# gaetanfacchinetti/DensityFlows.jl

Hardware: AMD Instinct MI355X
Metric: forward+logdetJ Msamples/s, d=5 8-layer RealNVP, 1/2/4/8 MI355X (higher is better)
Workload: dtype f32

## Files before the change

densityflows.jl_amd/csrc/df_uniform_impl.h:

```cpp
#pragma once

#include <type_traits>

#include "df_chain_impl.h"

namespace df {
namespace uni {


using impl::lds4;
using impl::mfma4;
using impl::Stager;

__device__ __forceinline__ float relu_fast(float x) {
    return __int_as_float(__builtin_elementwise_max(__float_as_int(x), 0));
}

__device__ __forceinline__ float xgroup_sum(float p) {
    auto a = __builtin_amdgcn_permlane16_swap(__float_as_uint(p), __float_as_uint(p), false, false);
    const float q = __uint_as_float(a[0]) + __uint_as_float(a[1]);
    auto b = __builtin_amdgcn_permlane32_swap(__float_as_uint(q), __float_as_uint(q), false, false);
    return __uint_as_float(b[0]) + __uint_as_float(b[1]);
}


template <int HT, int TT, int KS = 0>
__device__ __forceinline__ void dense_first(const uint8_t* buf, const UNet& N, const float (&xin)[TT][4],
                                            f32x4 (&acc)[TT][HT]) {
    const int lane = threadIdx.x & 63;
    const float* wb = reinterpret_cast<const float*>(buf + N.off_w0) + lane;
    const int ks = KS > 0 ? KS : N.ks;
    if constexpr (KS > 0) {
#pragma unroll
        for (int m = 0; m < HT; ++m) {
            const float w = wb[m * KS * 64];
#pragma unroll
            for (int t = 0; t < TT; ++t) acc[t][m] = mfma4(w, xin[t][0], f32x4{0.f, 0.f, 0.f, 0.f});
        }
#pragma unroll
        for (int r = 1; r < KS; ++r)
#pragma unroll
            for (int m = 0; m < HT; ++m) {
                const float w = wb[(m * KS + r) * 64];
#pragma unroll
                for (int t = 0; t < TT; ++t) acc[t][m] = mfma4(w, xin[t][r], acc[t][m]);
            }
        return;
    }
#pragma unroll
    for (int t = 0; t < TT; ++t)
#pragma unroll
        for (int m = 0; m < HT; ++m) acc[t][m] = f32x4{0.f, 0.f, 0.f, 0.f};
#pragma unroll
    for (int r = 0; r < 4; ++r) {
        if (r < ks) {
#pragma unroll
            for (int m = 0; m < HT; ++m) {
                const float w = wb[(m * ks + r) * 64];
#pragma unroll
                for (int t = 0; t < TT; ++t) acc[t][m] = mfma4(w, xin[t][r], acc[t][m]);
            }
        }
    }
}

template <int HT, int TT>
__device__ __forceinline__ void dense_hidden(const uint8_t* wb, const f32x4 (&in)[TT][HT], f32x4 (&out)[TT][HT]) {
    const int lane = threadIdx.x & 63;
    wb += lane * 16;
    constexpr int MB = HT < 2 ? HT : 2;
#pragma unroll
    for (int t = 0; t < TT; ++t)
#pragma unroll
        for (int m = 0; m < HT; ++m) out[t][m] = f32x4{0.f, 0.f, 0.f, 0.f};
#pragma unroll
    for (int m0 = 0; m0 < HT; m0 += MB) {
        f32x4 w[2][MB];
#pragma unroll
        for (int mm = 0; mm < MB; ++mm) w[0][mm] = lds4(wb + (m0 + mm) * 1024);
#pragma unroll
        for (int kq = 0; kq < HT; ++kq) {
            const int cb = kq & 1;
            if (kq + 1 < HT) {
#pragma unroll
                for (int mm = 0; mm < MB; ++mm) w[cb ^ 1][mm] = lds4(wb + ((kq + 1) * HT + m0 + mm) * 1024);
            }
#pragma unroll
            for (int r = 0; r < 4; ++r)
#pragma unroll
                for (int mm = 0; mm < MB; ++mm)
#pragma unroll
                    for (int t = 0; t < TT; ++t)
                        out[t][m0 + mm] = mfma4(w[cb][mm][r], in[t][kq][r], out[t][m0 + mm]);
        }
    }
}

template <int HT, int TT, bool RELU>
__device__ __forceinline__ void bias_act(const uint8_t* bb, int act, f32x4 (&v)[TT][HT], bool add_bias = true) {
    const int g = (threadIdx.x & 63) >> 4;
    if (add_bias) {
#pragma unroll
        for (int m = 0; m < HT; ++m) {
            const f32x4 b = lds4(bb + ((16 * m + 4 * g) << 2));
#pragma unroll
            for (int t = 0; t < TT; ++t) v[t][m] = v[t][m] + b;
        }
    }
    if (RELU || act == DF_ACT_RELU) {
#pragma unroll
        for (int t = 0; t < TT; ++t)
#pragma unroll
            for (int m = 0; m < HT; ++m)
#pragma unroll
                for (int r = 0; r < 4; ++r) v[t][m][r] = relu_fast(v[t][m][r]);
    } else if (act != DF_ACT_IDENTITY) {
        if (!RELU) {
#pragma unroll
            for (int t = 0; t < TT; ++t)
#pragma unroll
                for (int m = 0; m < HT; ++m)
#pragma unroll
                    for (int r = 0; r < 4; ++r) v[t][m][r] = impl::act_fn(act, v[t][m][r]);
        }
    }
}

template <int HT, int TT, bool RELU, int NO = 0>
__device__ __forceinline__ void out_valu(const uint8_t* buf, const UNet& N, const f32x4 (&h)[TT][HT],
                                         f32x4 (&o)[TT]) {
    const int g = (threadIdx.x & 63) >> 4;
    const uint8_t* w3 = buf + N.off_out;
    constexpr int INP = 16 * HT;
    const int n_out = NO > 0 ? NO : N.n_out;
    const float* b3 = reinterpret_cast<const float*>(w3) + n_out * INP;
#pragma unroll
    for (int t = 0; t < TT; ++t) o[t] = f32x4{0.f, 0.f, 0.f, 0.f};
#pragma unroll
    for (int oo = 0; oo < 4; ++oo) {
        if (oo < n_out) {
            float p[TT];
#pragma unroll
            for (int t = 0; t < TT; ++t) p[t] = 0.f;
#pragma unroll
            for (int kq = 0; kq < HT; ++kq) {
                const f32x4 w = lds4(w3 + ((oo * INP + 16 * kq + 4 * g) << 2));
#pragma unroll
                for (int r = 0; r < 4; ++r)
#pragma unroll
                    for (int t = 0; t < TT; ++t) p[t] = __builtin_fmaf(w[r], h[t][kq][r], p[t]);
            }
            const float bo = b3[oo];
#pragma unroll
            for (int t = 0; t < TT; ++t) {
                const float v = xgroup_sum(p[t]) + bo;
                o[t][oo] = (RELU || N.act_out == DF_ACT_IDENTITY) ? v : impl::act_fn(N.act_out, v);
            }
        }
    }
}

template <int HT, int TT, int NO>
__device__ __forceinline__ void out_valu_t(const uint8_t* buf, const UNet& N, const f32x4 (&h)[TT][HT],
                                           float (&y)[TT]) {
    static_assert(NO >= 1 && NO <= 4, "FAST tails: 1..4 outputs");
    const int g = (threadIdx.x & 63) >> 4;
    const uint8_t* w3 = buf + N.off_out;
    constexpr int INP = 16 * HT;
    float p[TT][4];
#pragma unroll
    for (int t = 0; t < TT; ++t)
#pragma unroll
        for (int oo = 0; oo < 4; ++oo) p[t][oo] = 0.f;
#pragma unroll
    for (int oo = 0; oo < NO; ++oo)
#pragma unroll
        for (int kq = 0; kq < HT; ++kq) {
            const f32x4 w = lds4(w3 + ((oo * INP + 16 * kq + 4 * g) << 2));
#pragma unroll
            for (int r = 0; r < 4; ++r)
#pragma unroll
                for (int t = 0; t < TT; ++t) p[t][oo] = __builtin_fmaf(w[r], h[t][kq][r], p[t][oo]);
        }
    const float bo = reinterpret_cast<const float*>(w3)[NO * INP + (g < NO ? g : 0)];
#pragma unroll
    for (int t = 0; t < TT; ++t) {
        auto a = __builtin_amdgcn_permlane16_swap(__float_as_uint(p[t][0]), __float_as_uint(p[t][1]), false, false);
        const float A = __uint_as_float(a[0]) + __uint_as_float(a[1]);
        float Bv = 0.f;
        if constexpr (NO > 2) {
            auto b = __builtin_amdgcn_permlane16_swap(__float_as_uint(p[t][2]), __float_as_uint(p[t][3]), false, false);
            Bv = __uint_as_float(b[0]) + __uint_as_float(b[1]);
        }
        auto c = __builtin_amdgcn_permlane32_swap(__float_as_uint(A), __float_as_uint(Bv), false, false);
        y[t] = (__uint_as_float(c[0]) + __uint_as_float(c[1])) + bo;
    }
}

template <int NO>
__device__ __forceinline__ float group_row_sum(float y) {
    float s = y;
    if constexpr (NO > 1) {
        auto a = __builtin_amdgcn_permlane16_swap(__float_as_uint(y), __float_as_uint(y), false, false);
        s = s + __uint_as_float(a[1]);
    }
    if constexpr (NO > 2) {
        auto b = __builtin_amdgcn_permlane32_swap(__float_as_uint(y), __float_as_uint(y), false, false);
        const float y2 = __uint_as_float(b[1]);
        s = s + y2;
        if constexpr (NO > 3) {
            auto c = __builtin_amdgcn_permlane16_swap(__float_as_uint(y2), __float_as_uint(y2), false, false);
            s = s + __uint_as_float(c[1]);
        }
    }
    return s;
}

template <int HT, int TT, bool RELU>
__device__ __forceinline__ void out_mfma(const uint8_t* buf, const UNet& N, const f32x4 (&h)[TT][HT],
                                         f32x4 (&out)[TT][2]) {
    const int lane = threadIdx.x & 63, g = lane >> 4;
    const uint8_t* wb = buf + N.off_out + lane * 16;
    const int mt = (N.n_out + 15) >> 4;
#pragma unroll
    for (int t = 0; t < TT; ++t) out[t][0] = out[t][1] = f32x4{0.f, 0.f, 0.f, 0.f};
#pragma unroll
    for (int kq = 0; kq < HT; ++kq) {
        const f32x4 w0 = lds4(wb + (kq * mt + 0) * 1024);
#pragma unroll
        for (int r = 0; r < 4; ++r)
#pragma unroll
            for (int t = 0; t < TT; ++t) out[t][0] = mfma4(w0[r], h[t][kq][r], out[t][0]);
        if (mt > 1) {
            const f32x4 w1 = lds4(wb + (kq * mt + 1) * 1024);
#pragma unroll
            for (int r = 0; r < 4; ++r)
#pragma unroll
                for (int t = 0; t < TT; ++t) out[t][1] = mfma4(w1[r], h[t][kq][r], out[t][1]);
        }
    }
    const uint8_t* bb = buf + N.off_out + HT * mt * 1024;
#pragma unroll
    for (int m = 0; m < 2; ++m) {
        if (m < mt) {
            const f32x4 b = lds4(bb + ((16 * m + 4 * g) << 2));
#pragma unroll
            for (int t = 0; t < TT; ++t) {
                f32x4 v = out[t][m] + b;
                if (!RELU && N.act_out != DF_ACT_IDENTITY)
#pragma unroll
                    for (int r = 0; r < 4; ++r) v[r] = impl::act_fn(N.act_out, v[r]);
                out[t][m] = v;
            }
        }
    }
}

template <int PH>
__device__ __forceinline__ float couple1(float v, float y) {
    if (PH == impl::PH_S_FWD) return v * expf(y);
    if (PH == impl::PH_T_FWD) return v + y;
    if (PH == impl::PH_T_BWD) return v - y;
    return v * expf(-y);
}

template <int HT, int TT, bool OUTV, bool RELU, int PH, int NO = 0>
__device__ __forceinline__ void tail(const uint8_t* buf, const UNet& N, const ULayer& L, const int32_t* tab,
                                     float* state, const int (&ro)[TT], float (&sum)[TT], const f32x4 (&H)[TT][HT]) {
    const int g = (threadIdx.x & 63) >> 4;
    constexpr bool SPH = (PH == impl::PH_S_FWD || PH == impl::PH_S_BWD);
    const int32_t* af = tab + L.af_tab;
    const int n_af = (OUTV && NO > 0) ? NO : L.n_af;
#pragma unroll
    for (int t = 0; t < TT; ++t) sum[t] = 0.f;
#ifdef DF_EXP_NOTAIL
    if (true) {
#pragma unroll
        for (int t = 0; t < TT; ++t) {
            float acc = 0.f;
#pragma unroll
            for (int m = 0; m < HT; ++m) acc += H[t][m][0];
            asm volatile("" ::"v"(acc));
        }
        return;
    }
#endif
    if constexpr (OUTV && NO > 0) {
        float y[TT];
        out_valu_t<HT, TT, NO>(buf, N, H, y);
        const int slot = af[g < NO ? g : 0];
#pragma unroll
        for (int t = 0; t < TT; ++t) {
            if (g < NO) state[ro[t] + slot] = couple1<PH>(state[ro[t] + slot], y[t]);
            if (SPH) sum[t] = group_row_sum<NO>(y[t]);
        }
    } else if constexpr (OUTV) {
        f32x4 o[TT];
        out_valu<HT, TT, RELU, NO>(buf, N, H, o);
        const int slot = (g < n_af) ? af[g] : 0;
#pragma unroll
        for (int t = 0; t < TT; ++t) {
            const float y = impl::sel4(o[t], g);
            if (g < n_af) state[ro[t] + slot] = couple1<PH>(state[ro[t] + slot], y);
            if (SPH) {
                float s_ = o[t][0];
#pragma unroll
                for (int oo = 1; oo < 4; ++oo)
                    if (oo < n_af) s_ = s_ + o[t][oo];
                sum[t] = s_;
            }
        }
    } else {
        f32x4 o[TT][2];
        out_mfma<HT, TT, RELU>(buf, N, H, o);
#pragma unroll
        for (int t = 0; t < TT; ++t) {
            float p = 0.f;
#pragma unroll
            for (int m = 0; m < 2; ++m)
#pragma unroll
                for (int r = 0; r < 4; ++r) {
                    const int oo = 16 * m + 4 * g + r;
                    if (oo < L.n_af) {
                        const int slot = af[oo];
                        const float y = o[t][m][r];
                        state[ro[t] + slot] = couple1<PH>(state[ro[t] + slot], y);
                        if (SPH) p = p + y;
                    }
                }
            if (SPH) sum[t] = xgroup_sum(p);
        }
    }
}

typedef __bf16 bf16x8 __attribute__((ext_vector_type(8)));

__device__ __forceinline__ f32x4 mfma_bf(const bf16x8& a, const bf16x8& b, f32x4 c) {
    return __builtin_amdgcn_mfma_f32_16x16x32_bf16(a, b, c, 0, 0, 0);
}

typedef __bf16 bf16x2 __attribute__((ext_vector_type(2)));
#ifndef DF_SPLIT_DOT2
#define DF_SPLIT_DOT2 1
#endif
template <int S>
__device__ __forceinline__ float split_rem(bf16x2 h, float x) {
#if DF_SPLIT_DOT2 == 2
    const uint32_t u = __builtin_bit_cast(uint32_t, h);
    const float hi = __uint_as_float(S == 0 ? (u << 16) : (u & 0xffff0000u));
    float r;
    asm("v_sub_f32 %0, %1, %2" : "=v"(r) : "v"(x), "v"(hi));
    return r;
#elif DF_SPLIT_DOT2
    uint32_t c;
    if (S == 0) asm("v_mov_b32 %0, 0xbf80" : "=v"(c));
    else c = 0xbf800000u;
    return __builtin_amdgcn_fdot2_f32_bf16(h, __builtin_bit_cast(bf16x2, c), x, false);
#else
    return x - (float)h[S];
#endif
}

__device__ __forceinline__ void split2(float a, float b, bf16x2& p0, bf16x2& p1, bf16x2& p2) {
    p0 = bf16x2{(__bf16)a, (__bf16)b};
    const float ra = split_rem<0>(p0, a), rb = split_rem<1>(p0, b);
    p1 = bf16x2{(__bf16)ra, (__bf16)rb};
    p2 = bf16x2{(__bf16)split_rem<0>(p1, ra), (__bf16)split_rem<1>(p1, rb)};
}

__device__ __forceinline__ void split8(const float (&v)[8], bf16x8& p0, bf16x8& p1, bf16x8& p2) {
#pragma unroll
    for (int e = 0; e < 8; e += 2) {
        bf16x2 h, m, l;
        split2(v[e], v[e + 1], h, m, l);
        p0[e] = h[0]; p0[e + 1] = h[1];
        p1[e] = m[0]; p1[e + 1] = m[1];
        p2[e] = l[0]; p2[e + 1] = l[1];
    }
}

#ifndef DF_SPLIT_MREM
#define DF_SPLIT_MREM 1
#endif
typedef short short4v __attribute__((ext_vector_type(4)));
typedef __bf16 bf16x4v __attribute__((ext_vector_type(4)));

__device__ __forceinline__ short4v neg_eye() {
    const int i = threadIdx.x & 3;
    short4v p;
#pragma unroll
    for (int e = 0; e < 4; ++e) p[e] = (e == i) ? (short)0xbf80 : (short)0;
    return p;
}

__device__ __forceinline__ f32x4 mrem(short4v eye, bf16x4v h, f32x4 c) {
    return __builtin_amdgcn_mfma_f32_4x4x4bf16_1k(eye, __builtin_bit_cast(short4v, h), c, 0, 0, 0);
}

__device__ __forceinline__ void split8_mrem(short4v eye, const f32x4& a, const f32x4& b, bf16x8& p0, bf16x8& p1,
                                            bf16x8& p2) {
    bf16x4v h0, h1;
#pragma unroll
    for (int e = 0; e < 4; ++e) {
        h0[e] = (__bf16)a[e];
        h1[e] = (__bf16)b[e];
    }
    p0 = __builtin_shufflevector(h0, h1, 0, 1, 2, 3, 4, 5, 6, 7);
    const f32x4 ra = mrem(eye, h0, a), rb = mrem(eye, h1, b);
#pragma unroll
    for (int e = 0; e < 4; ++e) {
        h0[e] = (__bf16)ra[e];
        h1[e] = (__bf16)rb[e];
    }
    p1 = __builtin_shufflevector(h0, h1, 0, 1, 2, 3, 4, 5, 6, 7);
    const f32x4 sa = mrem(eye, h0, ra), sb = mrem(eye, h1, rb);
#pragma unroll
    for (int e = 0; e < 4; ++e) {
        h0[e] = (__bf16)sa[e];
        h1[e] = (__bf16)sb[e];
    }
    p2 = __builtin_shufflevector(h0, h1, 0, 1, 2, 3, 4, 5, 6, 7);
}

template <int HT, int TT>
__device__ __forceinline__ void dense_first_split(const uint8_t* buf, const UNet& N, const float (&xin)[TT][4],
                                                  f32x4 (&acc)[TT][HT]) {
    const int lane = threadIdx.x & 63;
    bf16x8 b[TT];
    const __bf16 z = (__bf16)0.f;
#pragma unroll
    for (int t = 0; t < TT; t += 2) {
        bf16x2 h, m, l;
        split2(xin[t][0], t + 1 < TT ? xin[t + 1][0] : 0.f, h, m, l);
        b[t] = bf16x8{h[0], m[0], h[0], l[0], m[0], h[0], z, z};
        if (t + 1 < TT) b[t + 1] = bf16x8{h[1], m[1], h[1], l[1], m[1], h[1], z, z};
    }
    const uint8_t* wb = buf + N.off_w0 + lane * 16;
#pragma unroll
    for (int m = 0; m < HT; ++m) {
        const bf16x8 w = *reinterpret_cast<const bf16x8*>(wb + m * 1024);
#pragma unroll
        for (int t = 0; t < TT; ++t) acc[t][m] = mfma_bf(w, b[t], f32x4{0.f, 0.f, 0.f, 0.f});
    }
}

template <int HT, int TT, bool BIAS = true, bool FENCE = false>
__device__ __forceinline__ void dense_hidden_split(const uint8_t* wb, const f32x4 (&in)[TT][HT],
                                                   f32x4 (&out)[TT][HT]) {
    const int lane = threadIdx.x & 63, g = lane >> 4;
    const uint8_t* bb = wb + (HT / 2) * HT * 3072;
    wb += lane * 16;
    const short4v eye = DF_SPLIT_MREM ? neg_eye() : short4v{0, 0, 0, 0};
#pragma unroll
    for (int m = 0; m < HT; ++m) {
        const f32x4 b = BIAS ? lds4(bb + ((16 * m + 4 * g) << 2)) : f32x4{0.f, 0.f, 0.f, 0.f};
#pragma unroll
        for (int t = 0; t < TT; ++t) out[t][m] = b;
    }
#pragma unroll
    for (int c = 0; c < HT / 2; ++c) {
        bf16x8 x[TT][3];
#pragma unroll
        for (int t = 0; t < TT; ++t) {
            const float v[8] = {in[t][2 * c][0],     in[t][2 * c][1],     in[t][2 * c][2],     in[t][2 * c][3],
                                in[t][2 * c + 1][0], in[t][2 * c + 1][1], in[t][2 * c + 1][2], in[t][2 * c + 1][3]};
#ifdef DF_DIAG_NOSPLIT
            for (int e = 0; e < 8; ++e) x[t][0][e] = (__bf16)v[e];
            x[t][1] = x[t][0];
            x[t][2] = x[t][0];
#else
            if constexpr (DF_SPLIT_MREM) split8_mrem(eye, in[t][2 * c], in[t][2 * c + 1], x[t][0], x[t][1], x[t][2]);
            else split8(v, x[t][0], x[t][1], x[t][2]);
#endif
        }
#pragma unroll
        for (int m = 0; m < HT; ++m) {
            const uint8_t* f = wb + (c * HT + m) * 3072;
            const bf16x8 w0 = *reinterpret_cast<const bf16x8*>(f);
            const bf16x8 w1 = *reinterpret_cast<const bf16x8*>(f + 1024);
            const bf16x8 w2 = *reinterpret_cast<const bf16x8*>(f + 2048);
#pragma unroll
            for (int t = 0; t < TT; ++t) {
                f32x4 a = out[t][m];
                a = mfma_bf(w2, x[t][0], a);
                a = mfma_bf(w1, x[t][1], a);
                a = mfma_bf(w0, x[t][2], a);
                a = mfma_bf(w1, x[t][0], a);
                a = mfma_bf(w0, x[t][1], a);
                out[t][m] = mfma_bf(w0, x[t][0], a);
            }
            if (FENCE) asm volatile("" ::: "memory");
        }
    }
}

#ifndef DF_SPLIT_PREFETCH
#define DF_SPLIT_PREFETCH 1
#endif

__device__ __forceinline__ void sched_fence() { __builtin_amdgcn_sched_barrier(0); }

__device__ __forceinline__ void lds_wait0() { __builtin_amdgcn_s_waitcnt(0xc07f); }

struct SplitStep {
    bf16x8 w0, w1, w2;
    f32x4 b;
};

template <int HT, bool BIAS>
__device__ __forceinline__ void split_step_request(const uint8_t* wl, const uint8_t* bl, int s, SplitStep& f) {
    if (s >= (HT / 2) * HT) return;
    const uint8_t* p = wl + s * 3072;
    f.w0 = *reinterpret_cast<const bf16x8*>(p);
    f.w1 = *reinterpret_cast<const bf16x8*>(p + 1024);
    f.w2 = *reinterpret_cast<const bf16x8*>(p + 2048);
    if (BIAS && s < HT) f.b = lds4(bl + (s << 6));
}

template <int HT, int TT, bool BIAS = true>
__device__ __forceinline__ void dense_hidden_split_pf(const uint8_t* wb, int l16, int g16, const f32x4 (&in)[TT][HT],
                                                      f32x4 (&out)[TT][HT], const SplitStep& f0) {
    const uint8_t* bl = wb + (HT / 2) * HT * 3072 + g16;
    const uint8_t* wl = wb + l16;
    const short4v eye = neg_eye();
    SplitStep f[2];
    f[0] = f0;
    bf16x8 x[TT][3];
#pragma unroll
    for (int s = 0; s < (HT / 2) * HT; ++s) {
        const int c = s / HT, m = s % HT;
        if (m == 0) {
#pragma unroll
            for (int t = 0; t < TT; ++t) split8_mrem(eye, in[t][2 * c], in[t][2 * c + 1], x[t][0], x[t][1], x[t][2]);
        }
        constexpr int NS = (HT / 2) * HT;
        const bool late = (m == HT - 1) && (s + 1 < NS);
        sched_fence();
        lds_wait0();
        if (!late) split_step_request<HT, BIAS>(wl, bl, s + 1, f[(s + 1) & 1]);
        sched_fence();
        const SplitStep& w = f[s & 1];
#pragma unroll
        for (int t = 0; t < TT; ++t) {
            f32x4 a = c == 0 ? (BIAS ? w.b : f32x4{0.f, 0.f, 0.f, 0.f}) : out[t][m];
            a = mfma_bf(w.w2, x[t][0], a);
            a = mfma_bf(w.w1, x[t][1], a);
            a = mfma_bf(w.w0, x[t][2], a);
            a = mfma_bf(w.w1, x[t][0], a);
            a = mfma_bf(w.w0, x[t][1], a);
            out[t][m] = mfma_bf(w.w0, x[t][0], a);
        }
        if (late) {
#pragma unroll
            for (int t = 0; t < TT; ++t) asm volatile("" : "+v"(out[t][m]));
            sched_fence();
            split_step_request<HT, BIAS>(wl, bl, s + 1, f[(s + 1) & 1]);
        }
    }
}

template <int HT, int TT>
__device__ __forceinline__ void dense_first_split_pf(const bf16x8 (&w)[HT], const float (&xin)[TT][4],
                                                     f32x4 (&acc)[TT][HT]) {
    bf16x8 b[TT];
    const __bf16 z = (__bf16)0.f;
#pragma unroll
    for (int t = 0; t < TT; ++t) {
        bf16x2 h, m, l;
        h = bf16x2{(__bf16)xin[t][0], z};
        const float r1 = split_rem<0>(h, xin[t][0]);
        m = bf16x2{(__bf16)r1, z};
        l = bf16x2{(__bf16)split_rem<0>(m, r1), z};
        b[t] = bf16x8{h[0], m[0], h[0], l[0], m[0], h[0], z, z};
    }
#pragma unroll
    for (int m = 0; m < HT; ++m)
#pragma unroll
        for (int t = 0; t < TT; ++t) acc[t][m] = mfma_bf(w[m], b[t], f32x4{0.f, 0.f, 0.f, 0.f});
}

template <int HT, int NO>
__device__ __forceinline__ void out_row_request(const uint8_t* w3g, int oo, f32x4 (&w)[HT]) {
    if (oo >= NO) return;
#pragma unroll
    for (int kq = 0; kq < HT; ++kq) w[kq] = lds4(w3g + ((oo * 16 * HT + 16 * kq) << 2));
}

constexpr int split_tail_rows(int TT, int NO) { return (TT == 2 && NO <= 2) ? 1 : TT; }

template <int TT>
struct SplitTail {
    int ce, l16, g16;
    int row[TT];
    float e_old[TT], a_old[TT];
};

template <int HT, int TT, int NO, bool LDJ, int NU>
__device__ __forceinline__ void out_valu_t_pf(const uint8_t* w3g, const f32x4 (&w0)[HT], float bo,
                                              const f32x4 (&h)[TT][HT], const float* state, const int& aslot,
                                              SplitTail<TT>& tl, float (&v)[NU], float (&y)[NU]) {
    static_assert(NO >= 1 && NO <= 4, "FAST tails: 1..4 outputs");
    static_assert(NU == split_tail_rows(TT, NO), "rows a lane group owns");
    float p[TT][4];
#pragma unroll
    for (int t = 0; t < TT; ++t)
#pragma unroll
        for (int oo = 0; oo < 4; ++oo) p[t][oo] = 0.f;
    f32x4 w[2][HT];
#pragma unroll
    for (int kq = 0; kq < HT; ++kq) w[0][kq] = w0[kq];
#pragma unroll
    for (int oo = 0; oo < NO; ++oo) {
        sched_fence();
        lds_wait0();
        if (oo == 0) {
#pragma unroll
            for (int u = 0; u < NU; ++u) {
                v[u] = state[tl.row[u] + aslot];
                if constexpr (LDJ) {
                    tl.e_old[u] = state[tl.row[u] + tl.ce];
                    tl.a_old[u] = state[tl.row[u] + tl.ce - 1];
                }
            }
        }
        out_row_request<HT, NO>(w3g, oo + 1, w[(oo + 1) & 1]);
        sched_fence();
#pragma unroll
        for (int kq = 0; kq < HT; ++kq)
#pragma unroll
            for (int r = 0; r < 4; ++r)
#pragma unroll
                for (int t = 0; t < TT; ++t) p[t][oo] = __builtin_fmaf(w[oo & 1][kq][r], h[t][kq][r], p[t][oo]);
#pragma unroll
        for (int t = 0; t < TT; ++t) asm volatile("" : "+v"(p[t][oo]));
    }
    if constexpr (NU < TT) {
        const float q = NO == 2 ? p[0][1] : p[1][0];
        auto a = __builtin_amdgcn_permlane16_swap(__float_as_uint(p[0][0]), __float_as_uint(q), false, false);
        const float A = __uint_as_float(a[0]) + __uint_as_float(a[1]);
        float Bv = A;
        if constexpr (NO == 2) {
            auto b = __builtin_amdgcn_permlane16_swap(__float_as_uint(p[1][0]), __float_as_uint(p[1][1]), false, false);
            Bv = __uint_as_float(b[0]) + __uint_as_float(b[1]);
        }
        auto c = __builtin_amdgcn_permlane32_swap(__float_as_uint(A), __float_as_uint(Bv), false, false);
        y[0] = (__uint_as_float(c[0]) + __uint_as_float(c[1])) + bo;
    } else {
#pragma unroll
        for (int t = 0; t < TT; ++t) {
            auto a = __builtin_amdgcn_permlane16_swap(__float_as_uint(p[t][0]), __float_as_uint(p[t][1]), false, false);
            const float A = __uint_as_float(a[0]) + __uint_as_float(a[1]);
            float Bv = 0.f;
            if constexpr (NO > 2) {
                auto b = __builtin_amdgcn_permlane16_swap(__float_as_uint(p[t][2]), __float_as_uint(p[t][3]), false, false);
                Bv = __uint_as_float(b[0]) + __uint_as_float(b[1]);
            }
            auto c = __builtin_amdgcn_permlane32_swap(__float_as_uint(A), __float_as_uint(Bv), false, false);
            y[t] = (__uint_as_float(c[0]) + __uint_as_float(c[1])) + bo;
        }
    }
}

struct SplitHead {
    int off_w0, feat_word, af_word;
};
#if DF_SPLIT_PREFETCH && !defined(DF_EXP_NOTAIL) && !defined(DF_DIAG_NOSPLIT)
#define DF_SPLIT_HEAD_REGS 1
#else
#define DF_SPLIT_HEAD_REGS 0
#endif

#ifndef DF_SPLIT_PRIO
#define DF_SPLIT_PRIO 1
#endif
template <bool MATRIX_PHASE>
__device__ __forceinline__ void split_prio() {
    if constexpr (DF_SPLIT_PRIO == 1) __builtin_amdgcn_s_setprio(MATRIX_PHASE ? 2 : 0);
    if constexpr (DF_SPLIT_PRIO == 2) __builtin_amdgcn_s_setprio(MATRIX_PHASE ? 0 : 2);
}

template <int HT, int TT, bool OUTV, bool RELU, int PH, bool FAST = false, int NO = 0, bool SPLIT = false,
          bool LDJ = false, bool LANES = false>
__device__ __forceinline__ void net_tiles(const uint8_t* buf, const UNet& N, const ULayer& L, const int32_t* tab,
                                          float* state, const int (&ro)[TT], float (&sum)[TT], const SplitHead& hd,
                                          SplitTail<TT>& tl) {
    const int lane = threadIdx.x & 63, g = lane >> 4;
    constexpr bool SPH = (PH == impl::PH_S_FWD || PH == impl::PH_S_BWD);
#if DF_SPLIT_HEAD_REGS
    if constexpr (SPLIT && FAST && HT >= 2 && OUTV && NO > 0) {
        int l16 = tl.l16, g16 = tl.g16;
        if constexpr (!LANES) {
            int tx = threadIdx.x;
            asm volatile("" : "+v"(tx));
            l16 = (tx & 63) << 4, g16 = tx & 48;
        }
        const int g = g16 >> 4;
        const uint8_t* net = buf + hd.off_w0;
        const int slot = ((uint32_t)hd.feat_word >> (g16 >> 1)) & ((1 << kSplitSlotBits) - 1);
        static_assert(kSplitSlotBits == 8, "slot of lane group g at bit 8 g = g16 / 2");
        bf16x8 w0[HT];
#pragma unroll
        for (int m = 0; m < HT; ++m) w0[m] = *reinterpret_cast<const bf16x8*>(net + l16 + m * 1024);
        float xin[TT][4];
#pragma unroll
        for (int t = 0; t < TT; ++t) xin[t][0] = state[ro[t] + slot];
        const uint8_t* wh = net + kSplitOffH(HT);
        SplitStep f0;
        split_step_request<HT, true>(wh + l16, wh + (HT / 2) * HT * 3072 + g16, 0, f0);
        sched_fence();
        lds_wait0();
        split_prio<true>();
        sched_fence();
        f32x4 A[TT][HT], B[TT][HT];
        dense_first_split_pf<HT, TT>(w0, xin, A);
        bias_act<HT, TT, true>(buf, DF_ACT_RELU, A, false);
        dense_hidden_split_pf<HT, TT>(wh, l16, g16, A, B, f0);
        const uint8_t* w3 = net + kSplitOffOut(HT);
        const uint8_t* w3g = w3 + g16;
        sched_fence();
        split_prio<false>();
        f32x4 wo[HT];
        out_row_request<HT, NO>(w3g, 0, wo);
        constexpr int NU = split_tail_rows(TT, NO);
        constexpr bool ONE_TREE = NU < TT;
        const int go = ONE_TREE ? (NO == 2 ? (g & 1) : 0) : (g < NO ? g : 0);
        const float bo = reinterpret_cast<const float*>(w3)[NO * 16 * HT + go];
        const int aslot = ((uint32_t)hd.af_word >> (kSplitSlotBits * go)) & ((1 << kSplitSlotBits) - 1);
        if constexpr (ONE_TREE) {
            tl.row[0] = ro[0] + ((NO == 2 ? (g >> 1) : (g & 1)) ? ro[1] - ro[0] : 0);
        } else {
#pragma unroll
            for (int t = 0; t < TT; ++t) tl.row[t] = ro[t];
        }
        sched_fence();
        bias_act<HT, TT, true>(buf, DF_ACT_RELU, B, false);
        float v[NU], y[NU];
        out_valu_t_pf<HT, TT, NO, SPH && LDJ>(w3g, wo, bo, B, state, aslot, tl, v, y);
        if (ONE_TREE || g < NO) {
#pragma unroll
            for (int u = 0; u < NU; ++u) state[tl.row[u] + aslot] = couple1<PH>(v[u], y[u]);
        }
#pragma unroll
        for (int u = 0; u < NU; ++u) {
            if constexpr (!SPH) {
                sum[u] = 0.f;
            } else if constexpr (ONE_TREE && NO == 2) {
                auto a = __builtin_amdgcn_permlane16_swap(__float_as_uint(y[u]), __float_as_uint(y[u]), false, false);
                sum[u] = __uint_as_float(a[0]) + __uint_as_float(a[1]);
            } else if constexpr (ONE_TREE) {
                sum[u] = y[u];
            } else {
                sum[u] = group_row_sum<NO>(y[u]);
            }
        }
        return;
    }
#endif
    if constexpr (SPLIT && FAST && HT >= 2) {
        float xin[TT][4];
        const int slot = tab[L.feat_tab + g];
#pragma unroll
        for (int t = 0; t < TT; ++t) xin[t][0] = state[ro[t] + slot];
        f32x4 A[TT][HT], B[TT][HT];
        dense_first_split<HT, TT>(buf, N, xin, A);
        bias_act<HT, TT, true>(buf, DF_ACT_RELU, A, false);
        dense_hidden_split<HT, TT>(buf + N.off_h, A, B);
        bias_act<HT, TT, true>(buf, DF_ACT_RELU, B, false);
        tail<HT, TT, OUTV, RELU, PH, NO>(buf, N, L, tab, state, ro, sum, B);
        return;
    }
    float xin[TT][4];
    const int32_t* feat = tab + L.feat_tab;
    constexpr int KS = FAST ? 1 : 0;
    const int ks = FAST ? 1 : N.ks;
#pragma unroll
    for (int r = 0; r < 4; ++r) {
        const int slot = (r < ks) ? feat[4 * r + g] : 0;
#pragma unroll
        for (int t = 0; t < TT; ++t) xin[t][r] = (r < ks) ? state[ro[t] + slot] : 0.f;
    }

    f32x4 A[TT][HT], B[TT][HT];
    dense_first<HT, TT, KS>(buf, N, xin, A);
    bias_act<HT, TT, RELU>(buf + N.off_b0, N.act0, A, FAST ? false : !N.fold0);
    if (FAST || N.nh == 1) {
        dense_hidden<HT, TT>(buf + N.off_h, A, B);
        bias_act<HT, TT, RELU>(buf + N.off_h + HT * HT * 1024, N.acth, B);
        tail<HT, TT, OUTV, RELU, PH, NO>(buf, N, L, tab, state, ro, sum, B);
        return;
    }
    bool in_a = true;
    for (int k = 0; k < N.nh; k += 2) {
        dense_hidden<HT, TT>(buf + N.off_h + k * N.hstride, A, B);
        bias_act<HT, TT, RELU>(buf + N.off_h + k * N.hstride + HT * HT * 1024, N.acth, B);
        in_a = false;
        if (k + 1 < N.nh) {
            dense_hidden<HT, TT>(buf + N.off_h + (k + 1) * N.hstride, B, A);
            bias_act<HT, TT, RELU>(buf + N.off_h + (k + 1) * N.hstride + HT * HT * 1024, N.acth, A);
            in_a = true;
        }
    }
    if (in_a) tail<HT, TT, OUTV, RELU, PH, NO>(buf, N, L, tab, state, ro, sum, A);
    else tail<HT, TT, OUTV, RELU, PH, NO>(buf, N, L, tab, state, ro, sum, B);
}

template <int HT, int TT, bool RELU, bool FWDP, int NO>
__device__ __forceinline__ void net_pair_tiles(const uint8_t* buf, const ULayer& L, const int32_t* tab, float* state,
                                               const int (&ro)[TT], float (&ssum)[TT]) {
    const int lane = threadIdx.x & 63, g = lane >> 4;
    float xin[TT][4];
    const int slot_in = tab[L.feat_tab + g];
#pragma unroll
    for (int t = 0; t < TT; ++t) xin[t][0] = state[ro[t] + slot_in];
    f32x4 As[TT][HT], At[TT][HT], Bs[TT][HT], Bt[TT][HT];
    dense_first<HT, TT, 1>(buf, L.s, xin, As);
    dense_first<HT, TT, 1>(buf, L.t, xin, At);
    bias_act<HT, TT, RELU>(buf + L.s.off_b0, L.s.act0, As, false);
    bias_act<HT, TT, RELU>(buf + L.t.off_b0, L.t.act0, At, false);
    dense_hidden<HT, TT>(buf + L.s.off_h, As, Bs);
    dense_hidden<HT, TT>(buf + L.t.off_h, At, Bt);
    bias_act<HT, TT, RELU>(buf + L.s.off_h + HT * HT * 1024, L.s.acth, Bs);
    bias_act<HT, TT, RELU>(buf + L.t.off_h + HT * HT * 1024, L.t.acth, Bt);
    float ys[TT], yt[TT];
    out_valu_t<HT, TT, NO>(buf, L.s, Bs, ys);
    out_valu_t<HT, TT, NO>(buf, L.t, Bt, yt);
    const int slot = tab[L.af_tab + (g < NO ? g : 0)];
#pragma unroll
    for (int t = 0; t < TT; ++t) {
        if (g < NO) {
            float v = state[ro[t] + slot];
            if (FWDP) {
                v = v * expf(ys[t]);
                v = v + yt[t];
            } else {
                v = v - yt[t];
                v = v * expf(-ys[t]);
            }
            state[ro[t] + slot] = v;
        }
        ssum[t] = group_row_sum<NO>(ys[t]);
    }
}

}

#ifndef DF_UNI_WAVES
#define DF_UNI_WAVES 4
#endif
#ifndef DF_FAST_WAVES
#define DF_FAST_WAVES 4
#endif

template <int HT, int MODE, bool OUTV, bool RELU, bool FAST = false, bool SPLIT = false>
__global__ void __launch_bounds__(kBlockThreads, FAST ? DF_FAST_WAVES : DF_UNI_WAVES)
uniform_kernel(ChainArgs a) {
    using namespace uni;
    constexpr bool FWD = (MODE == MODE_FWD || MODE == MODE_FWD_INPLACE);
    constexpr bool WANT_LDJ = (MODE != MODE_FWD_INPLACE);

    extern __shared__ __attribute__((aligned(16))) uint8_t smem[];
    const int stage_area = a.stage_bytes * a.n_stage_bufs;
    int32_t* tab = reinterpret_cast<int32_t*>(smem + stage_area);
    float* state = reinterpret_cast<float*>(smem + stage_area + a.tab_bytes);

    ClockStamp clk;
    clk.begin(a);
#ifdef DF_PHASE_STAMPS
    uint64_t ph[16] = {};
#define DF_PH(i) do { if (blockIdx.x == 0 && threadIdx.x == 0) ph[i] = __builtin_amdgcn_s_memtime(); } while (0)
#else
#define DF_PH(i) do {} while (0)
#endif
    DF_PH(0);
    const int tid = threadIdx.x;
    const int lane = tid & 63, wave = tid >> 6;
    const int g = lane >> 4, j = lane & 15;
    const int d = a.d, n = a.n, stride = a.stride, nd = n + d;
    const int nt = a.tiles;
    const int S = kWavesPerBlock * 16 * nt;
    const int cA = nd + 1, cE = nd + 2;
    const int64_t s0 = (int64_t)blockIdx.x * S;
    const int nvalid = (int)((a.batch - s0) < S ? (a.batch - s0) : S);

    Stager sg;
    sg.base = smem;
    sg.bytes = a.stage_bytes;
    sg.sched = FWD ? a.sched_fwd : a.sched_bwd;
    sg.n = FWD ? a.n_sched_fwd : a.n_sched_bwd;
    constexpr bool kLaneLocalDma = SPLIT && DF_SPLIT_PREFETCH;
    constexpr bool kSplitHead = SPLIT && FAST && OUTV && HT >= 2 && DF_SPLIT_HEAD_REGS;
    impl::stager_start<kLaneLocalDma>(sg, a);

    float* tabf = reinterpret_cast<float*>(tab);
    constexpr int kRowMax = 8;
    const bool fast_copy = d <= kRowMax && n <= kRowMax && a.n_par <= kBlockThreads && a.tab_ints <= 4 * kBlockThreads;
    auto row_init = [&](int smp) {
        for (int c = nd; c < stride; ++c) state[smp * stride + c] = (c == nd + 3) ? 1.f : 0.f;
    };
    auto theta_in = [&](float v, float lo, float hi) {
        const float diff = hi - lo;
        return (diff == 0.f) ? 0.f : (v - lo) / diff;
    };
    if (fast_copy) {
        const int n_tab = a.tab_ints, n_par = a.n_par;
        int tv[4];
#pragma unroll
        for (int u = 0; u < 4; ++u) {
            const int i = tid + u * kBlockThreads;
            tv[u] = i < n_tab ? a.tables[i] : 0;
        }
        const float pv = tid < n_par ? a.params[tid] : 0.f;
        const bool norm_th = a.tmin != nullptr;
        const float blo = (norm_th && lane < n) ? a.tmin[lane] : 0.f;
        const float bhi = (norm_th && lane < n) ? a.tmax[lane] : 0.f;
        const int smp = tid;
        const bool valid = smp < nvalid;
        float zr[kRowMax], tr[kRowMax];
#pragma unroll
        for (int c = 0; c < kRowMax; ++c)
            if (c < d) zr[c] = valid ? a.zin[(s0 + smp) * d + c] : 0.f;
#pragma unroll
        for (int c = 0; c < kRowMax; ++c)
            if (c < n) tr[c] = valid ? a.theta[(s0 + smp) * n + c] : 0.f;
#pragma unroll
        for (int u = 0; u < 4; ++u) {
            const int i = tid + u * kBlockThreads;
            if (i < n_tab) tab[i] = tv[u];
        }
        if (tid < n_par) tabf[n_tab + tid] = pv;
#pragma unroll
        for (int c = 0; c < kRowMax; ++c)
            if (c < n) {
                const float lo = __shfl(blo, c), hi = __shfl(bhi, c);
                if (smp < S) state[smp * stride + c] = (norm_th && valid) ? theta_in(tr[c], lo, hi) : tr[c];
            }
        if (smp < S) {
#pragma unroll
            for (int c = 0; c < kRowMax; ++c)
                if (c < d) state[smp * stride + n + c] = zr[c];
            row_init(smp);
        }
        for (int i = tid + kBlockThreads * d; i < S * d; i += kBlockThreads) {
            const int r = i / d, c = i - r * d;
            state[r * stride + n + c] = r < nvalid ? a.zin[(s0 + r) * d + c] : 0.f;
        }
        for (int i = tid + kBlockThreads * n; i < S * n; i += kBlockThreads) {
            const int r = i / n, c = i - r * n;
            float v = 0.f;
            if (r < nvalid) {
                v = a.theta[(s0 + r) * n + c];
                if (norm_th) v = theta_in(v, a.tmin[c], a.tmax[c]);
            }
            state[r * stride + c] = v;
        }
        for (int r = tid + kBlockThreads; r < S; r += kBlockThreads) row_init(r);
    } else {
        for (int i = tid; i < a.tab_ints; i += kBlockThreads) tab[i] = a.tables[i];
        for (int i = tid; i < S * d; i += kBlockThreads) {
            const int smp = i / d, c = i - smp * d;
            float v = 0.f;
            if (smp < nvalid) v = a.zin[(s0 + smp) * d + c];
            state[smp * stride + n + c] = v;
        }
        for (int i = tid; i < S * n; i += kBlockThreads) {
            const int smp = i / n, c = i - smp * n;
            float v = 0.f;
            if (smp < nvalid) {
                v = a.theta[(s0 + smp) * n + c];
                if (a.tmin) v = theta_in(v, a.tmin[c], a.tmax[c]);
            }
            state[smp * stride + c] = v;
        }
        for (int i = tid; i < S; i += kBlockThreads) row_init(i);
    }
    DF_PH(1);
    DF_PH(2);
    DF_PH(3);
    __syncthreads();
    DF_PH(4);

    const int row0 = ((wave * nt) * 16 + j) * stride;
#ifdef DF_NO_PAIR
    constexpr bool no_pair = true;
#else
    constexpr bool no_pair = false;
#endif
    const int tstep = 16 * stride;
    bool have_acc = false;
    constexpr bool kHoldLanes = kSplitHead && HT == 4 && FWD;
    int lane16 = lane << 4, group16 = g << 4;
    if constexpr (kHoldLanes) asm volatile("" : "+v"(lane16), "+v"(group16));

    auto ldj_update = [&](int ro, float l, bool first_in_elem, bool last_in_elem) {
        if (!WANT_LDJ || g != 0) return;
        const float e = first_in_elem ? l : state[ro + cE] + l;
        state[ro + cE] = e;
        if (last_in_elem) state[ro + cA] = have_acc ? state[ro + cA] + e : e;
    };

    for (int it = 0; it < a.n_layers; ++it) {
        const int li = FWD ? it : a.n_layers - 1 - it;
        using CULayer = const __attribute__((address_space(4))) ULayer;
#ifdef DF_PHASE_STAMPS
        const ULayer L = *(const ULayer*)(&((CULayer*)(uintptr_t)a.ulayers)[li]);
        asm volatile("s_waitcnt lgkmcnt(0)" ::: "memory");
        if (it == 1) DF_PH(13);
#else
        const ULayer& L = *(const ULayer*)(&((CULayer*)(uintptr_t)a.ulayers)[li]);
#endif
        const int kind = L.kind;
        const bool first_in_elem = FWD ? L.elem_start : L.elem_end;
        const bool last_in_elem = FWD ? L.elem_end : L.elem_start;
        int gl = g, jl = j, wavel = wave, row0l = row0;
        if constexpr (kLaneLocalDma) {
            if (kind == DF_LAYER_NORM || (!FWD && a.snap)) {
                int tx = tid;
                asm volatile("" : "+v"(tx));
                gl = (tx & 63) >> 4, jl = tx & 15, wavel = tx >> 6;
                row0l = ((wavel * nt) * 16 + jl) * stride;
            }
        }
        if (kind == DF_LAYER_NORM) {
            const float al = L.alpha, be = L.beta, delta = be - al;
            auto norm = [&](const auto* xmn) {
                const auto* xmx = xmn + d;
                for (int tt = 0; tt < nt; ++tt) {
                    const int ro = row0l + tt * tstep;
                    for (int i = gl; i < d; i += 4) {
                        const float lo = xmn[i], hi = xmx[i], xd = hi - lo;
                        float v = state[ro + n + i];
                        if (FWD) v = ((xd * v - al * hi) + be * lo) / delta;
                        else v = (be * (v - lo) + al * (hi - v)) / xd;
                        state[ro + n + i] = v;
                    }
                    ldj_update(ro, FWD ? L.ldj_const : -L.ldj_const, first_in_elem, last_in_elem);
                }
            };
            if (fast_copy) norm(tabf + a.tab_ints + L.norm_off);
            else norm(a.params + L.norm_off);
        } else {
            const bool rnvp = (kind == DF_LAYER_RNVP);
            constexpr int kTT = FAST ? kFastTileGroup : kUniformTileGroup;
            auto tiles_loop = [&](const UNet& N, const SplitHead& hd, auto ph_tag, auto no_tag, bool sphase,
                                  float sign) {
                constexpr int PH = decltype(ph_tag)::value;
                constexpr int NO = decltype(no_tag)::value;
                const uint8_t* buf = sg.buf();
                for (int tt = 0; tt < nt; tt += kTT) {
                    int ro[kTT];
                    float ssum[kTT];
                    int r0 = row0;
                    if constexpr (SPLIT) asm volatile("" : "+v"(r0));
#pragma unroll
                    for (int t = 0; t < kTT; ++t) ro[t] = r0 + (tt + t) * tstep;
                    SplitTail<kTT> tl;
                    tl.ce = cE, tl.l16 = lane16, tl.g16 = group16;
                    net_tiles<HT, kTT, OUTV, RELU, PH, FAST, NO, SPLIT, WANT_LDJ, kHoldLanes>(buf, N, L, tab, state, ro,
                                                                                              ssum, hd, tl);
                    constexpr bool SPH = (PH == impl::PH_S_FWD || PH == impl::PH_S_BWD);
                    if constexpr (kSplitHead && NO > 0 && SPH) {
                        constexpr int NU = split_tail_rows(kTT, NO);
                        if constexpr (WANT_LDJ) {
                            if (NU < kTT || g == 0) {
#pragma unroll
                                for (int u = 0; u < NU; ++u) {
                                    const float l = sign * ssum[u];
                                    const float e = first_in_elem ? l : tl.e_old[u] + l;
                                    state[tl.row[u] + cE] = e;
                                    if (last_in_elem) state[tl.row[u] + cA] = have_acc ? tl.a_old[u] + e : e;
                                }
                            }
                        }
                    } else {
#pragma unroll
                        for (int t = 0; t < kTT; ++t) {
                            if (sphase) ldj_update(ro[t], sign * ssum[t], first_in_elem, last_in_elem);
                            else if (!rnvp) ldj_update(ro[t], 0.f, first_in_elem, last_in_elem);
                        }
                    }
                }
            };
            auto run_net = [&](const UNet& N, auto ph_tag, bool sphase, float sign) {
                SplitHead hd{0, 0, 0};
                int stage = N.stage, n_out = N.n_out;
                if constexpr (kSplitHead) {
                    hd = SplitHead{N.off_w0, L.feat_word, L.af_word};
                    asm volatile("" : "+s"(stage), "+s"(n_out), "+s"(hd.off_w0), "+s"(hd.feat_word), "+s"(hd.af_word));
                }
                impl::ensure_stage<kLaneLocalDma>(stage, sg, a);
                if constexpr (FAST && OUTV) {
                    switch (n_out) {
                        case 1: tiles_loop(N, hd, ph_tag, std::integral_constant<int, 1>{}, sphase, sign); break;
                        case 2: tiles_loop(N, hd, ph_tag, std::integral_constant<int, 2>{}, sphase, sign); break;
                        case 3: tiles_loop(N, hd, ph_tag, std::integral_constant<int, 3>{}, sphase, sign); break;
                        default: tiles_loop(N, hd, ph_tag, std::integral_constant<int, 4>{}, sphase, sign); break;
                    }
                } else {
                    tiles_loop(N, hd, ph_tag, std::integral_constant<int, 0>{}, sphase, sign);
                }
            };
            using PSF = std::integral_constant<int, impl::PH_S_FWD>;
            using PTF = std::integral_constant<int, impl::PH_T_FWD>;
            using PTB = std::integral_constant<int, impl::PH_T_BWD>;
            using PSB = std::integral_constant<int, impl::PH_S_BWD>;
            bool paired = false;
            if constexpr (FAST && OUTV && !SPLIT && HT <= 2) {
                if (rnvp && L.s.stage == L.t.stage && L.s.n_out == L.t.n_out && !no_pair) {
                    impl::ensure_stage(L.s.stage, sg, a);
                    auto pair_loop = [&](auto no_tag) {
                        constexpr int NO = decltype(no_tag)::value;
                        const uint8_t* buf = sg.buf();
                        for (int tt = 0; tt < nt; tt += kTT) {
                            int ro[kTT];
                            float ssum[kTT];
#pragma unroll
                            for (int t = 0; t < kTT; ++t) ro[t] = row0 + (tt + t) * tstep;
                            net_pair_tiles<HT, kTT, RELU, FWD, NO>(buf, L, tab, state, ro, ssum);
#pragma unroll
                            for (int t = 0; t < kTT; ++t)
                                ldj_update(ro[t], FWD ? ssum[t] : -ssum[t], first_in_elem, last_in_elem);
                        }
                    };
                    switch (L.s.n_out) {
                        case 1: pair_loop(std::integral_constant<int, 1>{}); break;
                        case 2: pair_loop(std::integral_constant<int, 2>{}); break;
                        case 3: pair_loop(std::integral_constant<int, 3>{}); break;
                        default: pair_loop(std::integral_constant<int, 4>{}); break;
                    }
                    paired = true;
                }
            }
            if (paired) {
            } else if (FWD) {
#ifdef DF_PHASE_STAMPS
                if (it == 1) DF_PH(11);
#endif
                if (rnvp) run_net(L.s, PSF{}, true, 1.f);
#ifdef DF_PHASE_STAMPS
                if (it == 1) DF_PH(12);
#endif
                run_net(L.t, PTF{}, false, 1.f);
            } else {
                run_net(L.t, PTB{}, false, 1.f);
                if (rnvp) run_net(L.s, PSB{}, true, -1.f);
            }
        }
        have_acc = have_acc || last_in_elem;
#ifdef DF_PHASE_STAMPS
        if (it == 0) DF_PH(5);
        if (it == 1) DF_PH(6);
        if (it == 2) DF_PH(7);
        if (it == 3) DF_PH(8);
#endif
        if (!FWD && a.snap) {
            float* dst = a.snap + (int64_t)li * a.batch * d;
            for (int tt = 0; tt < nt; ++tt) {
                const int smp = (wavel * nt + tt) * 16 + jl;
                if (smp < nvalid)
                    for (int i = gl; i < d; i += 4) dst[(s0 + smp) * d + i] = state[row0l + tt * tstep + n + i];
            }
        }
    }

    asm volatile("s_waitcnt vmcnt(0)" ::: "memory");
    if (MODE == MODE_LOGPDF) {
        double part = 0.0;
        if (g == 0) {
            for (int tt = 0; tt < nt; ++tt) {
                const int ro = row0 + tt * tstep;
                const int smp = (wave * nt + tt) * 16 + j;
                float q = 0.f;
                for (int i = 0; i < d; ++i) {
                    const float zz = state[ro + n + i];
                    q = q + zz * zz;
                }
                const float lp = (a.c0 - q / 2.f) + state[ro + cA];
                if (smp < nvalid) {
                    if (a.lp_out) a.lp_out[s0 + smp] = lp;
                    part += (double)lp;
                }
            }
        }
        if (a.partial) {
#pragma unroll
            for (int off = 32; off >= 1; off >>= 1) part += __shfl_xor(part, off);
            __syncthreads();
            double* red = reinterpret_cast<double*>(smem);
            if (lane == 0) red[wave] = part;
            __syncthreads();
            if (tid == 0) {
                double s = 0.0;
                for (int w = 0; w < kWavesPerBlock; ++w) s += red[w];
                a.partial[blockIdx.x] = s;
            }
        }
        if (!a.xout) {
            clk.end(a);
            return;
        }
    }
    __syncthreads();
    for (int i = tid; i < S * d; i += kBlockThreads) {
        const int smp = i / d, c = i - smp * d;
        if (smp < nvalid) a.xout[(s0 + smp) * d + c] = state[smp * stride + n + c];
    }
    if (WANT_LDJ && MODE != MODE_LOGPDF && a.ldj_out) {
        for (int i = tid; i < nvalid; i += kBlockThreads) a.ldj_out[s0 + i] = state[i * stride + cA];
    }
    DF_PH(9);
#ifdef DF_PHASE_STAMPS
    asm volatile("s_waitcnt vmcnt(0)" ::: "memory");
    DF_PH(10);
    if (blockIdx.x == 0 && threadIdx.x == 0) {
#pragma unroll
        for (int i = 1; i < 14; ++i) a.xout[i] = (float)(ph[i] - ph[0]);
    }
#endif
#undef DF_PH
    clk.end(a);
}

template <int HT, bool RELU, bool FAST = false, bool SPLIT = false>
void* uniform_kernel_ptr_r(int mode, bool outv) {
#define DF_U(M) (outv ? reinterpret_cast<void*>(&uniform_kernel<HT, M, true, RELU, FAST, SPLIT>) \
                      : reinterpret_cast<void*>(&uniform_kernel<HT, M, false, RELU, FAST, SPLIT>))
    switch (mode) {
        case MODE_FWD: return DF_U(MODE_FWD);
        case MODE_FWD_INPLACE: return DF_U(MODE_FWD_INPLACE);
        case MODE_BWD: return DF_U(MODE_BWD);
        default: return DF_U(MODE_LOGPDF);
    }
#undef DF_U
}

template <int HT>
void* uniform_kernel_ptr(int mode, int variant) {
    const bool outv = variant & 1;
    if constexpr (HT >= 2) {
        if ((variant & 8) && (variant & 4) && outv) return uniform_kernel_ptr_r<HT, true, true, true>(mode, true);
    }
    if (variant & 8) return nullptr;
    if (variant & 4) return uniform_kernel_ptr_r<HT, true, true>(mode, outv);
    return (variant & 2) ? uniform_kernel_ptr_r<HT, true>(mode, outv) : uniform_kernel_ptr_r<HT, false>(mode, outv);
}

template <int HT>
hipError_t launch_uniform_ht(int mode, int variant, const ChainArgs& a, unsigned grid, size_t lds, hipStream_t st) {
    void* args[] = {const_cast<ChainArgs*>(&a)};
    return hipLaunchKernel(uniform_kernel_ptr<HT>(mode, variant), dim3(grid), dim3(kBlockThreads), args, lds, st);
}

template <int HT>
hipError_t set_uniform_lds_limit_ht(size_t lds) {
    for (int mode = 0; mode < 4; ++mode)
        for (int v = 0; v < 16; ++v) {
            void* k = uniform_kernel_ptr<HT>(mode, v);
            if (!k) continue;
            hipError_t e = hipFuncSetAttribute(k,
                                               hipFuncAttributeMaxDynamicSharedMemorySize, (int)lds);
            if (e != hipSuccess) return e;
        }
    return hipSuccess;
}

template <int HT>
hipError_t uniform_occupancy_ht(int mode, int variant, size_t lds, int* blocks) {
    return hipOccupancyMaxActiveBlocksPerMultiprocessor(blocks, uniform_kernel_ptr<HT>(mode, variant), kBlockThreads,
                                                        lds);
}

}
```

Before: 1675.

## Extend paired-row split tail to 3-4 output coupling nets when holding lanes

Generalizes the split-head output tail so that, with two tiles and held lanes, each lane group handles outputs of both rows through combined permlane reduction trees, instead of only when there are at most two outputs. Bias, slot and log-det column indexing become per-value arrays, with tile-step offsets folded into the state addresses. The first-layer bf16 split packing is also restructured to build the mid/high pair in one packed register. This aims to cut redundant cross-lane reduction and idle lane groups in the output tail, at the cost of more complex indexing and ownership logic for the log-det writes.

```diff
diff --git a/densityflows.jl_amd/csrc/df_uniform_impl.h b/densityflows.jl_amd/csrc/df_uniform_impl.h
--- a/densityflows.jl_amd/csrc/df_uniform_impl.h
+++ b/densityflows.jl_amd/csrc/df_uniform_impl.h
@@ -566,12 +566,13 @@
     const __bf16 z = (__bf16)0.f;
 #pragma unroll
     for (int t = 0; t < TT; ++t) {
-        bf16x2 h, m, l;
-        h = bf16x2{(__bf16)xin[t][0], z};
+        const bf16x2 h = bf16x2{(__bf16)xin[t][0], z};
         const float r1 = split_rem<0>(h, xin[t][0]);
-        m = bf16x2{(__bf16)r1, z};
-        l = bf16x2{(__bf16)split_rem<0>(m, r1), z};
-        b[t] = bf16x8{h[0], m[0], h[0], l[0], m[0], h[0], z, z};
+        uint32_t w = __builtin_bit_cast(uint32_t, bf16x2{(__bf16)r1, (__bf16)xin[t][0]});
+        asm("" : "+v"(w));
+        const bf16x2 mh = __builtin_bit_cast(bf16x2, w);
+        const __bf16 l = (__bf16)split_rem<0>(mh, r1);
+        b[t] = bf16x8{(__bf16)xin[t][0], (__bf16)r1, (__bf16)xin[t][0], l, mh[0], mh[1], z, z};
     }
 #pragma unroll
     for (int m = 0; m < HT; ++m)
@@ -586,21 +587,35 @@
     for (int kq = 0; kq < HT; ++kq) w[kq] = lds4(w3g + ((oo * 16 * HT + 16 * kq) << 2));
 }
 
-constexpr int split_tail_rows(int TT, int NO) { return (TT == 2 && NO <= 2) ? 1 : TT; }
+constexpr bool split_tail_pair(int TT, int NO, bool WIDE) { return TT == 2 && (NO <= 2 || WIDE); }
+constexpr int split_tail_vals(int TT, int NO, bool WIDE) { return split_tail_pair(TT, NO, WIDE) ? (NO + 1) / 2 : TT; }
+constexpr int split_tail_rows(int TT, int NO, bool WIDE) { return split_tail_pair(TT, NO, WIDE) ? 1 : TT; }
+
+__device__ __forceinline__ float pair_tree(float a0, float a1, float b0, float b1) {
+    auto a = __builtin_amdgcn_permlane16_swap(__float_as_uint(a0), __float_as_uint(a1), false, false);
+    const float A = __uint_as_float(a[0]) + __uint_as_float(a[1]);
+    auto b = __builtin_amdgcn_permlane16_swap(__float_as_uint(b0), __float_as_uint(b1), false, false);
+    const float Bv = __uint_as_float(b[0]) + __uint_as_float(b[1]);
+    auto c = __builtin_amdgcn_permlane32_swap(__float_as_uint(A), __float_as_uint(Bv), false, false);
+    return __uint_as_float(c[0]) + __uint_as_float(c[1]);
+}
 
 template <int TT>
 struct SplitTail {
-    int ce, l16, g16;
+    int ce, ts, l16, g16;
+    int lcol;
     int row[TT];
     float e_old[TT], a_old[TT];
 };
 
-template <int HT, int TT, int NO, bool LDJ, int NU>
-__device__ __forceinline__ void out_valu_t_pf(const uint8_t* w3g, const f32x4 (&w0)[HT], float bo,
-                                              const f32x4 (&h)[TT][HT], const float* state, const int& aslot,
+template <int HT, int TT, int NO, bool LDJ, bool WIDE, int NU>
+__device__ __forceinline__ void out_valu_t_pf(const uint8_t* w3g, const f32x4 (&w0)[HT], const float (&bo)[NU],
+                                              const f32x4 (&h)[TT][HT], const float* state, const int (&aslot)[NU],
                                               SplitTail<TT>& tl, float (&v)[NU], float (&y)[NU]) {
     static_assert(NO >= 1 && NO <= 4, "FAST tails: 1..4 outputs");
-    static_assert(NU == split_tail_rows(TT, NO), "rows a lane group owns");
+    static_assert(NU == split_tail_vals(TT, NO, WIDE), "outputs a lane group owns");
+    constexpr bool PAIR = split_tail_pair(TT, NO, WIDE);
+    constexpr int NR = split_tail_rows(TT, NO, WIDE);
     float p[TT][4];
 #pragma unroll
     for (int t = 0; t < TT; ++t)
@@ -615,11 +630,12 @@
         lds_wait0();
         if (oo == 0) {
 #pragma unroll
-            for (int u = 0; u < NU; ++u) {
-                v[u] = state[tl.row[u] + aslot];
-                if constexpr (LDJ) {
-                    tl.e_old[u] = state[tl.row[u] + tl.ce];
-                    tl.a_old[u] = state[tl.row[u] + tl.ce - 1];
+            for (int u = 0; u < NU; ++u) v[u] = state[tl.row[NR == 1 ? 0 : u] + aslot[u]];
+            if constexpr (LDJ) {
+#pragma unroll
+                for (int r = 0; r < NR; ++r) {
+                    tl.e_old[r] = state[tl.row[r] + tl.lcol];
+                    tl.a_old[r] = state[tl.row[r] + tl.lcol - 1];
                 }
             }
         }
@@ -634,7 +650,17 @@
 #pragma unroll
         for (int t = 0; t < TT; ++t) asm volatile("" : "+v"(p[t][oo]));
     }
-    if constexpr (NU < TT) {
+    if constexpr (PAIR && NO >= 3) {
+        y[0] = pair_tree(p[0][0], p[0][1], p[1][0], p[1][1]) + bo[0];
+        if constexpr (NO == 4) {
+            y[1] = pair_tree(p[0][2], p[0][3], p[1][2], p[1][3]) + bo[1];
+        } else {
+            auto a = __builtin_amdgcn_permlane16_swap(__float_as_uint(p[0][2]), __float_as_uint(p[1][2]), false, false);
+            const float A = __uint_as_float(a[0]) + __uint_as_float(a[1]);
+            auto c = __builtin_amdgcn_permlane32_swap(__float_as_uint(A), __float_as_uint(A), false, false);
+            y[1] = (__uint_as_float(c[0]) + __uint_as_float(c[1])) + bo[1];
+        }
+    } else if constexpr (PAIR) {
         const float q = NO == 2 ? p[0][1] : p[1][0];
         auto a = __builtin_amdgcn_permlane16_swap(__float_as_uint(p[0][0]), __float_as_uint(q), false, false);
         const float A = __uint_as_float(a[0]) + __uint_as_float(a[1]);
@@ -644,7 +670,7 @@
             Bv = __uint_as_float(b[0]) + __uint_as_float(b[1]);
         }
         auto c = __builtin_amdgcn_permlane32_swap(__float_as_uint(A), __float_as_uint(Bv), false, false);
-        y[0] = (__uint_as_float(c[0]) + __uint_as_float(c[1])) + bo;
+        y[0] = (__uint_as_float(c[0]) + __uint_as_float(c[1])) + bo[0];
     } else {
 #pragma unroll
         for (int t = 0; t < TT; ++t) {
@@ -656,7 +682,7 @@
                 Bv = __uint_as_float(b[0]) + __uint_as_float(b[1]);
             }
             auto c = __builtin_amdgcn_permlane32_swap(__float_as_uint(A), __float_as_uint(Bv), false, false);
-            y[t] = (__uint_as_float(c[0]) + __uint_as_float(c[1])) + bo;
+            y[t] = (__uint_as_float(c[0]) + __uint_as_float(c[1])) + bo[t];
         }
     }
 }
@@ -721,37 +747,62 @@
         split_prio<false>();
         f32x4 wo[HT];
         out_row_request<HT, NO>(w3g, 0, wo);
-        constexpr int NU = split_tail_rows(TT, NO);
-        constexpr bool ONE_TREE = NU < TT;
-        const int go = ONE_TREE ? (NO == 2 ? (g & 1) : 0) : (g < NO ? g : 0);
-        const float bo = reinterpret_cast<const float*>(w3)[NO * 16 * HT + go];
-        const int aslot = ((uint32_t)hd.af_word >> (kSplitSlotBits * go)) & ((1 << kSplitSlotBits) - 1);
-        if constexpr (ONE_TREE) {
-            tl.row[0] = ro[0] + ((NO == 2 ? (g >> 1) : (g & 1)) ? ro[1] - ro[0] : 0);
+        constexpr int NU = split_tail_vals(TT, NO, LANES);
+        constexpr int NR = split_tail_rows(TT, NO, LANES);
+        constexpr bool PAIR = split_tail_pair(TT, NO, LANES);
+        const float* bias = reinterpret_cast<const float*>(w3) + NO * 16 * HT;
+        float bo[NU];
+        int aslot[NU];
+        tl.lcol = tl.ce;
+        if constexpr (PAIR) {
+            const int go = NO == 1 ? 0 : (g & 1);
+            const int t0 = (NO == 1 ? (g & 1) : (g >> 1)) ? tl.ts : 0;
+            bo[0] = bias[go];
+            aslot[0] = (((uint32_t)hd.af_word >> (kSplitSlotBits * go)) & ((1 << kSplitSlotBits) - 1)) + t0;
+            tl.lcol = tl.ce + t0;
+            if constexpr (NO == 3) {
+                bo[1] = bias[2];
+                aslot[1] = (((uint32_t)hd.af_word >> (kSplitSlotBits * 2)) & ((1 << kSplitSlotBits) - 1)) +
+                           (go ? tl.ts : 0);
+            } else if constexpr (NO == 4) {
+                bo[1] = bias[go + 2];
+                aslot[1] = (((uint32_t)hd.af_word >> (kSplitSlotBits * (go + 2))) & ((1 << kSplitSlotBits) - 1)) + t0;
+            }
+            tl.row[0] = ro[0];
         } else {
-#pragma unroll
-            for (int t = 0; t < TT; ++t) tl.row[t] = ro[t];
+            const int go = g < NO ? g : 0;
+#pragma unroll
+            for (int t = 0; t < TT; ++t) {
+                bo[t] = bias[go];
+                aslot[t] = ((uint32_t)hd.af_word >> (kSplitSlotBits * go)) & ((1 << kSplitSlotBits) - 1);
+                tl.row[t] = ro[t];
+            }
         }
         sched_fence();
         bias_act<HT, TT, true>(buf, DF_ACT_RELU, B, false);
         float v[NU], y[NU];
-        out_valu_t_pf<HT, TT, NO, SPH && LDJ>(w3g, wo, bo, B, state, aslot, tl, v, y);
-        if (ONE_TREE || g < NO) {
-#pragma unroll
-            for (int u = 0; u < NU; ++u) state[tl.row[u] + aslot] = couple1<PH>(v[u], y[u]);
-        }
-#pragma unroll
-        for (int u = 0; u < NU; ++u) {
-            if constexpr (!SPH) {
-                sum[u] = 0.f;
-            } else if constexpr (ONE_TREE && NO == 2) {
-                auto a = __builtin_amdgcn_permlane16_swap(__float_as_uint(y[u]), __float_as_uint(y[u]), false, false);
-                sum[u] = __uint_as_float(a[0]) + __uint_as_float(a[1]);
-            } else if constexpr (ONE_TREE) {
-                sum[u] = y[u];
-            } else {
-                sum[u] = group_row_sum<NO>(y[u]);
-            }
+        out_valu_t_pf<HT, TT, NO, SPH && LDJ, LANES>(w3g, wo, bo, B, state, aslot, tl, v, y);
+        if (PAIR || g < NO) {
+#pragma unroll
+            for (int u = 0; u < NU; ++u) state[tl.row[NR == 1 ? 0 : u] + aslot[u]] = couple1<PH>(v[u], y[u]);
+        }
+        if constexpr (!SPH) {
+#pragma unroll
+            for (int t = 0; t < TT; ++t) sum[t] = 0.f;
+        } else if constexpr (PAIR && NO == 1) {
+            sum[0] = y[0];
+        } else if constexpr (PAIR) {
+            auto a = __builtin_amdgcn_permlane16_swap(__float_as_uint(y[0]), __float_as_uint(y[0]), false, false);
+            float s = __uint_as_float(a[0]) + __uint_as_float(a[1]);
+            if constexpr (NO == 3) s = s + y[1];
+            if constexpr (NO == 4) {
+                auto c = __builtin_amdgcn_permlane16_swap(__float_as_uint(y[1]), __float_as_uint(y[1]), false, false);
+                s = (s + __uint_as_float(c[0])) + __uint_as_float(c[1]);
+            }
+            sum[0] = s;
+        } else {
+#pragma unroll
+            for (int t = 0; t < TT; ++t) sum[t] = group_row_sum<NO>(y[t]);
         }
         return;
     }
@@ -1054,20 +1105,21 @@
 #pragma unroll
                     for (int t = 0; t < kTT; ++t) ro[t] = r0 + (tt + t) * tstep;
                     SplitTail<kTT> tl;
-                    tl.ce = cE, tl.l16 = lane16, tl.g16 = group16;
+                    tl.ce = cE, tl.ts = tstep, tl.l16 = lane16, tl.g16 = group16;
                     net_tiles<HT, kTT, OUTV, RELU, PH, FAST, NO, SPLIT, WANT_LDJ, kHoldLanes>(buf, N, L, tab, state, ro,
                                                                                               ssum, hd, tl);
                     constexpr bool SPH = (PH == impl::PH_S_FWD || PH == impl::PH_S_BWD);
                     if constexpr (kSplitHead && NO > 0 && SPH) {
-                        constexpr int NU = split_tail_rows(kTT, NO);
+                        constexpr bool PAIR = split_tail_pair(kTT, NO, kHoldLanes);
+                        constexpr int NU = split_tail_rows(kTT, NO, kHoldLanes);
                         if constexpr (WANT_LDJ) {
-                            if (NU < kTT || g == 0) {
+                            if (PAIR ? (NO != 3 || g == 0 || g == 3) : g == 0) {
 #pragma unroll
                                 for (int u = 0; u < NU; ++u) {
                                     const float l = sign * ssum[u];
                                     const float e = first_in_elem ? l : tl.e_old[u] + l;
-                                    state[tl.row[u] + cE] = e;
-                                    if (last_in_elem) state[tl.row[u] + cA] = have_acc ? tl.a_old[u] + e : e;
+                                    state[tl.row[u] + tl.lcol] = e;
+                                    if (last_in_elem) state[tl.row[u] + tl.lcol - 1] = have_acc ? tl.a_old[u] + e : e;
                                 }
                             }
                         }
```

Measured after the change: 1693, median of 6. +1.1%, better.
